# rrwick/Polypolish

Hardware: AMD Instinct MI355X
Metric: assembly Mbp polished/sec at 200x coverage; bit-identical FASTA vs reference (higher is better)
Workload: dtype u8/u32 counts + f64 depth

## Files before the change

polypolish_amd/__init__.py:

```python
from __future__ import annotations

import ctypes as C
import os

import numpy as np

HERE = os.path.dirname(os.path.abspath(__file__))
ROOT = os.path.dirname(HERE)
LIB_PATH = os.environ.get("PP_LIB_PATH") or os.path.join(HERE, "_build", "libpolypolish_hip.so")

OK, ERR_QUIT, ERR_HIP, ERR_ARG, ERR_LIMIT, ERR_PANIC = 0, 1, 3, 4, 5, 101
ERR_NOT_ASCII = 6
MEM_HOST, MEM_DEVICE, MEM_PEER = 0, 1, 2
STATUS = ("kept", "changed", "low_depth", "none", "multiple", "too_close")
OPS = "MIDNSHP=X"


class PolypolishError(RuntimeError):
    def __init__(self, code, msg):
        super().__init__(f"[{code}] {msg}")
        self.code, self.msg = code, msg


class Params(C.Structure):
# ... 1002 lines not shown
        run._keep = keep
        return run

    def result_size(self):
        n = C.c_uint64()
        self._chk(lib().pp_polish_result_size(self._h, C.byref(n)))
        return n.value

    def result_device_ptr(self):
        return lib().pp_polish_result_device(self._h)

    def result(self):
        n = self.result_size()
        out = np.zeros(max(n, 1), dtype=np.uint8)
        offs = np.zeros(self._n_contigs + 1, dtype=np.uint64)
        stats = (ContigStats * self._n_contigs)()
        self._chk(lib().pp_polish_result(self._h, out.ctypes.data, MEM_HOST, offs.ctypes.data, stats))
        st = [dict(polished_len=s.polished_len, changed=s.changed, zero_depth=s.zero_depth, depth_sum=s.depth_sum)
              for s in stats]
        return out[:n].tobytes(), offs, st

    def trust_mirrors(self, on=True):
        f = lib().pp_ctx_trust_mirrors_
        f.argtypes = [C.c_void_p, C.c_int]
        f.restype = C.c_int
        self._chk(f(self._h, int(bool(on))))

    def took_direct_path(self):
        return bool(lib().pp_polish_took_direct_path(self._h))

    def kernel_times(self):
        kt = KernelTimes()
        lib().pp_polish_kernel_times(self._h, C.byref(kt))
        return kt.as_dict()

    def first_kernel_ms(self):
        kt = getattr(self, "_kt", None)
        if kt is None:
            kt = self._kt = KernelTimes()
            self._kt_ref = C.byref(kt)
            self._kt_fn = lib().pp_polish_kernel_times
        self._kt_fn(self._h, self._kt_ref)
        return (kt.name[0], kt.ms[0]) if kt.n else None

    def positions(self):
        G = self._G
        arrs = {"depth": np.zeros(G, np.float64), "status": np.zeros(G, np.uint8)}
        for k in ("count_a", "count_c", "count_g", "count_t", "count_other", "valid_thr", "invalid_thr"):
            arrs[k] = np.zeros(G, np.uint32)
        po = PositionsOut(*[arrs[k].ctypes.data for k in ("depth", "count_a", "count_c", "count_g", "count_t",
                                                          "count_other", "valid_thr", "invalid_thr", "status")])
        self._chk(lib().pp_polish_positions(self._h, C.byref(po)))
        return arrs

    def debug_tsv(self, contig_names, lo=0, hi=None, chunk=64 << 20) -> bytes:
        names = [n.encode() if isinstance(n, str) else bytes(n) for n in contig_names]
        if len(names) != self._n_contigs:
            raise PolypolishError(ERR_ARG, "debug_tsv: one name per contig")
        arr = (C.c_char_p * max(len(names), 1))(*names)
        hi = self._G if hi is None else int(hi)
        buf = np.empty(max(int(chunk), 1), dtype=np.uint8)
        n, nxt = C.c_uint64(), C.c_uint64()
        parts, p = [], int(lo)
        while True:
            self._chk(lib().pp_polish_debug_tsv(self._h, C.cast(arr, C.c_void_p), p, hi, buf.ctypes.data, MEM_HOST, len(buf),
                                                C.byref(n), C.byref(nxt)))
            parts.append(buf[:n.value].tobytes())
# ... 130 lines not shown
```

polypolish_amd/csrc/pp_internal.h:

```cpp
#pragma once

#include <hip/hip_runtime.h>

#include <cstdarg>
#include <cstdint>
#include <cstdio>
#include <string>
#include <thread>
#include <vector>

#include "polypolish_hip.h"

#ifndef PP_MIRROR_REGISTRY_DECLARED
#define PP_MIRROR_REGISTRY_DECLARED
void pp_mirror_register_(const void *owner, const void *p, size_t bytes);
void pp_mirror_forget_(const void *owner);
bool pp_mirror_trusted_(const void *p, size_t bytes);
#endif

namespace pp {

constexpr int TILE = 2048;
constexpr int TILE_THREADS = 1024;
constexpr int COARSE_WINDOWS = 8;
// ... 28 lines not shown
    DE_LEN_MISMATCH = 2,
    DE_OUT_OF_BOUNDS = 3,
    DE_BAD_CONTIG = 4,
    DE_BAD_K = 5,
    DE_BAD_RUN = 6,
    DE_BAD_ENDS = 7,
    DE_NON_ASCII = 8,
    DE_INTERNAL = 9,
    DE_TOO_DEEP = 10,
    DE_OVERFLOW = 11,
    DE_CAPACITY = 12,
    DE_HALO = 14,
    DE_CAPACITY_LATE = 13,
    DE_BAD_MIRROR = 15,
    DE_MIRROR_ORDER = 16,
    DE_SEQ_RANGE = 18,
    DE_GW_HINT = 17,
};


enum MetaWord : uint32_t {
    MW_STATUS = 0,
    MW_COUNTERS = 1,
    MW_ITEMS = 3,
    MW_SCRATCH = 4,
    MW_OUT_BYTES = 5,
    MW_REPLAY_ITEMS = 6,
    MW_KEYS = 8,
    MW_MAXLEN = 9,
    MW_SCR_NEED = 10,
    MW_X_NEED = 12,
    MW_N_NEED = 13,
    MW_XMAT_ITEMS = 14,
    MW_CTG_OUT = 16,
};
enum MetaCounter : uint32_t {
    MC_LISTED = 0,
    MC_MULTI = 1,
    MC_FLAGGED = 2,
    MC_SLABS = 3,
};
constexpr size_t meta_stats_at(size_t nc) { return (size_t)MW_CTG_OUT + nc + 1; }
constexpr size_t meta_heavy_at(size_t nc) { return meta_stats_at(nc) + 3 * nc; }
constexpr size_t meta_words(size_t nc) { return meta_heavy_at(nc) + (HEAVY_WORDS + 1) / 2; }

struct MetaView {
    const uint64_t *w;
    uint64_t operator[](MetaWord i) const { return w[i]; }
    uint32_t counter(MetaCounter c) const { return (uint32_t)(w[MW_COUNTERS + c / 2] >> (32 * (c & 1))); }
    bool ok() const { return w[MW_STATUS] == ~0ull; }
};

struct DevBuf {
    void *p = nullptr;
    size_t cap = 0;
};

struct KernelTimer {
    const char *name;
    hipEvent_t start, stop;
};

struct ContigStatsDev {
    unsigned long long changed;
    unsigned long long zero_depth;
    unsigned long long depth_fx;
// ... 20 lines not shown
    uint32_t n_contigs = 0;
    std::vector<uint64_t> contig_off;
    uint64_t G = 0;
    pp_params params{};
    const uint8_t *d_bases = nullptr;
    pp_aln_batch dbatch{};
    bool have_batch = false;
    bool batch_borrowed = false;
    uint64_t acc_n = 0, acc_seq = 0, acc_cig = 0;
    uint64_t total_out = 0, n_multi = 0, n_keys = 0;
    uint64_t last_dev_error = ~0ull;
    std::vector<uint64_t> contig_out_off;
    std::vector<pp_contig_stats> stats;

    pp::DevBuf b_bases, b_contig_off, b_status;
    pp::DevBuf b_in[11];
    bool acc_wo = false;
    pp::DevBuf b_gstart, b_nkeep, b_aflag, b_hist, b_wincnt, b_winoff, b_entA, b_entB, b_ccnt, b_coff;
    pp::DevBuf b_code, b_winlen, b_winout, b_flag_pos, b_flag_cov, b_flag_scr, b_scratch;
    pp::DevBuf b_vote_tab;
    pp::DevBuf b_multi, b_meta, b_out, b_flag_bits, b_win_nflag, b_win_slab, b_slab_win, b_slabs, b_ents, b_keys, b_own;
    pp::DevBuf b_win_heavy, b_hslab;
    std::vector<uint64_t> wo_runs;
    pp::DevBuf b_runs, b_first, b_xcnt, b_xent, b_need_win, b_win_lo, b_win_hi;
    std::vector<uint32_t> runs_on_dev;
    size_t xcap = 0;
    bool no_direct = false;
    bool wo_untrusted = false;
    bool trust_all = false;
    bool no_wo = false;
    size_t xcap_limit = ~(size_t)0;
    uint32_t maxlen_hint = 0;
    bool last_direct = false;
    bool nothing_flagged_last = false;
    std::vector<uint32_t> emit;
    std::vector<uint32_t> run_full_of;
    uint32_t run_nc = 0;
    uint32_t last_multi = ~0u;
    uint32_t last_listed = ~0u;
    bool no_compact = false;
    uint64_t *h_meta = nullptr;
    pp::DevBuf b_wincoarse;
    pp::DevBuf b_emit_done;
    bool emit_done_clean = false;
    uint64_t *d_hmeta = nullptr;
    bool stream_may_be_busy = false;
    uint64_t emit_serial = 0;
    struct MetaReady {
        const void *meta; uint32_t words; const void *za, *zb, *zc; uint32_t nwin; const void *tab; double fv, fi; const void *ze;
        bool operator==(const MetaReady &o) const {
            return meta == o.meta && words == o.words && za == o.za && zb == o.zb && zc == o.zc && nwin == o.nwin && tab == o.tab && fv == o.fv && fi == o.fi && ze == o.ze;
        }
    };
    MetaReady meta_ready{};
    bool meta_ready_valid = false;
    size_t h_meta_words = 0;
    std::vector<uint8_t> own_blob;
    pp::DevBuf b_sub_bases;
    size_t cap_ent = 0, cap_scr = 0, cap_multi = 0, cap_out = 0, cap_flag = 0, cap_slabs = 0, cap_ents = 0, cap_keys = 0;
    pp::DevBuf b_dbg_depth, b_dbg_counts, b_dbg_status;
    bool job_debug = false;
    bool dfmt_ready = false;
    pp::DevBuf b_dfmt_idx, b_dfmt_rec;
    pp::DevBuf b_dfmt_names, b_dfmt_noff, b_dfmt_emit;
    pp::DevBuf b_dfmt_len, b_dfmt_bsum, b_dfmt_boff, b_dfmt_res, b_dfmt_stage;

// ... 45 lines not shown
```

polypolish_amd/csrc/pp_k_direct.h:

```cpp
#pragma once

#include "pp_wo_home.h"

namespace pp {

constexpr u32 NOHOME = 0xFFFFFFFFu;
__device__ __forceinline__ bool wo_bulk(bool contig_ok, u32 ref_start, u32 seq_len, u32 op0, u64 clen) {
    return contig_ok && op0 == ((seq_len << 4) | (u32)PP_OP_M) && seq_len > 0 && seq_len <= FAST_MAX_LEN && (u64)ref_start + seq_len <= clen;
}
__device__ __forceinline__ uint4 wo_item(u64 so, u32 len, u32 kc, u64 g, u32 w, u32 file_idx) {
    uint4 e;
    e.x = (u32)so;
    e.y = ((u32)(so >> 32) & 0xFFu) | (kc << 8) | (len << 24);
    e.z = (u32)(int)((long long)g - (long long)w * TILE) & 0x3FFFFFFFu;
    e.w = file_idx;
    return e;
}

constexpr u32 XLOCAL = 64, CTG_LDS = 1024;
struct CtgTab {
    const u64 *lds, *mem;
    bool in_lds;
    __device__ __forceinline__ u64 operator()(u32 i) const {
        u32 x, y;
        if (in_lds) {
            const u64 v = lds[i];
            x = (u32)v; y = (u32)(v >> 32);
            asm volatile("" : "+v"(x), "+v"(y));
        } else {
            const u64 v = mem[i];
            x = (u32)v; y = (u32)(v >> 32);
            asm volatile("" : "+v"(x), "+v"(y));
        }
        return (u64)x | ((u64)y << 32);
    }
    __device__ __forceinline__ void pair(u32 i, u64 &a, u64 &b) const {
        u32 x, y, z, w;
        if (in_lds) {
            const u64 v = lds[i], v1 = lds[i + 1u];
            x = (u32)v; y = (u32)(v >> 32); z = (u32)v1; w = (u32)(v1 >> 32);
            asm volatile("" : "+v"(x), "+v"(y), "+v"(z), "+v"(w));
        } else {
            const u64 v = mem[i], v1 = mem[i + 1u];
            x = (u32)v; y = (u32)(v >> 32); z = (u32)v1; w = (u32)(v1 >> 32);
            asm volatile("" : "+v"(x), "+v"(y), "+v"(z), "+v"(w));
        }
        a = (u64)x | ((u64)y << 32);
        b = (u64)z | ((u64)w << 32);
    }
};
struct XSink {
    uint4 *st_item;
    u32 *st_key;
    u32 *l_cnt, *l_base, *l_nb;
    u32 *n_st;
    u32 xstage, wbase, xcap;
    u32 *x_cnt, *x_nb;
    uint4 *xent;
    u64 *x_need, *status;
    __device__ __forceinline__ void put(u32 w, u32 slot, const uint4 &e) const {
        if (slot < xcap) xent[(u64)w * xcap + slot] = e;
        else {
            atomicMax(x_need, (u64)slot + 1ull);
            report(status, slot, DE_CAPACITY);
        }
    }
    __device__ __forceinline__ void emit(u32 w, const uint4 &e) const {
        const u32 wl = w - wbase;
        if (wl < XLOCAL) {
            const u32 pos = atomicAdd(n_st, 1u);
            if (pos < xstage) {
                st_key[pos] = (wl << 16) | atomicAdd(&l_cnt[wl], 1u);
                st_item[pos] = e;
                return;
            }
        }
        put(w, atomicAdd(&x_cnt[w], 1u), e);
    }
    __device__ __forceinline__ void not_bulk(u32 h) const {
        if (h - wbase < XLOCAL) atomicAdd(&l_nb[h - wbase], 1u); else atomicAdd(&x_nb[h], 1u);
    }
    __device__ __forceinline__ void clear() const {
        if (threadIdx.x < XLOCAL) { l_cnt[threadIdx.x] = 0; l_nb[threadIdx.x] = 0; }
        if (threadIdx.x == 0) *n_st = 0;
    }
    __device__ __forceinline__ void flush() const {
        __syncthreads();
        if (threadIdx.x < XLOCAL) {
            const u32 c = l_cnt[threadIdx.x], nb = l_nb[threadIdx.x];
            l_base[threadIdx.x] = c ? atomicAdd(&x_cnt[wbase + threadIdx.x], c) : 0u;
            if (nb) atomicAdd(&x_nb[wbase + threadIdx.x], nb);
        }
        __syncthreads();
        for (u32 i = threadIdx.x; i < min(*n_st, xstage); i += blockDim.x) {
            const u32 key = st_key[i], wl = key >> 16;
            put(wbase + wl, l_base[wl] + (key & 0xFFFFu), st_item[i]);
        }
    }
};

struct PrepdArgs {
    u64 n;
    const pp_wo_rec *wo;
    const u64 *cig_off;
    const u32 *n_cig, *cigar;
    const u8 *seq;
    const u64 *contig_off;
    u32 n_contigs, nwin;
    const u32 *run_end;
    u32 n_runs;
    u32 *first, *x_cnt, *x_nb;
    uint4 *xent;
    u32 xcap;
    u32 *maxlen;
    u64 *x_need;
    u64 unused_[3];
    u64 seq_bytes;
    u64 *status;
};

template <typename CTG>
__device__ __forceinline__ void general_record(const pp_wo_rec &r, const PrepdArgs &P, CTG ctg, const XSink &X) {
    u32 g_out = 0, nk_out = 0;
    u8 fl_out = 0;
    const u32 fi = r.file_idx;
    if (fi >= P.n) return;
    if (r.contig >= P.n_contigs) { report(P.status, fi, DE_BAD_CONTIG); return; }
    const u64 c_lo = ctg(r.contig), c_hi = ctg(r.contig + 1u);
    X.not_bulk(wo_home(c_lo, r.ref_start, P.nwin));
    {
        const bool multi = r.op0 == PP_WO_MULTI_RUN;
        const u32 sl = r.seq_len;
        const u8 *const sq = P.seq + r.seq_off;
        u64 tail8 = 0;
        if (sl >= 8u) __builtin_memcpy(&tail8, sq + (sl - 8u), 8);
        u32 nc = 1;
        u64 co = 0;
        if (multi) { nc = P.n_cig[fi]; co = P.cig_off[fi]; }
        if (nc == 0) report(P.status, fi, DE_BAD_RUN);
        else {
            const u32 *const cg = P.cigar + co;
            u32 r0 = r.op0, r1 = 0, r2 = 0, r3 = 0, r4 = 0, r5 = 0, r6 = 0, r7 = 0;
            if (multi) {
                r0 = cg[0];
                r1 = cg[min(1u, nc - 1u)]; r2 = cg[min(2u, nc - 1u)]; r3 = cg[min(3u, nc - 1u)]; r4 = cg[min(4u, nc - 1u)];
                r5 = cg[min(5u, nc - 1u)]; r6 = cg[min(6u, nc - 1u)]; r7 = cg[min(7u, nc - 1u)];
            }
            prep_general_t(fi, r.ref_start, sl, nc,
                           [&](u32 i) -> u32 {
// ... 1 lines not shown
                               const u32 a = (i & 1u) ? r1 : r0, b = (i & 1u) ? r3 : r2, c = (i & 1u) ? r5 : r4, d = (i & 1u) ? r7 : r6;
                               const u32 ab = (i & 2u) ? b : a, cd = (i & 2u) ? d : c;
                               return (i & 4u) ? cd : ab;
                           },
                           [&](u32 i) -> u8 { return sl >= 8u && i + 8u >= sl ? (u8)(tail8 >> (8u * (i + 8u - sl))) : sq[i]; },
                           c_lo, c_hi - c_lo, &g_out, &nk_out, &fl_out, P.status);
        }
    }
    const u32 word = nk_out | ((u32)fl_out << 30);
    if (!word) return;
    const u32 kc = kclass_of(r.k);
    const u32 cls = word >> 30, ia = (word >> 9) & 0xFFu, idel = (word >> 17) & 1u;
    for_each_piece(g_out, word, [&](u32 piece, u32 g, u32 sp) {
        if (!sp) return;
        const u32 wa = g / (u32)TILE, wb = min((g + sp - 1u) / (u32)TILE, P.nwin - 1u);
        u64 pso = r.seq_off;
        u32 len = sp, fl = 0, zf = 0;
        if (cls == NKW_INDEL1) {
            if (piece == 0u) zf = 1u;
            else if (piece == 1u) { zf = 2u; pso += ia - 1u + idel; len = idel ? 0u : 2u; }
            else pso += idel ? ia : ia + 1u;
        } else fl = cls;
        for (u32 w = wa; w <= wb && w >= wa; w++) {
            uint4 e;
            e.x = fl ? sp : (u32)pso;
            e.y = (fl ? 0u : (((u32)(pso >> 32) & 0xFFu) | (len << 24))) | (kc << 8) | (fl << 16);
            e.z = ((u32)(int)((long long)g - (long long)w * TILE) & 0x3FFFFFFFu) | (zf << 30);
            e.w = fi;
            X.emit(w, e);
        }
    });
}

template <int THREADS>
__global__ __launch_bounds__(THREADS, PP_PREP_WAVES) void k_prepd(u64 chunk, PrepdArgs P) {
    constexpr u32 LATER_MAX = THREADS >= 1024 ? 768 : 320, XSTAGE = 2 * THREADS;
    __shared__ uint4 later[2 * LATER_MAX];
    __shared__ u32 n_later, s_unit;
    __shared__ uint4 st_item[XSTAGE];
    __shared__ u32 st_key[XSTAGE], l_cnt[XLOCAL], l_base[XLOCAL], l_nb[XLOCAL], n_st, s_wbase;
    __shared__ u64 s_ctg[CTG_LDS + 1];
    PP_STAMP(0, 0);
    const u64 n = P.n;
    const pp_wo_rec *const wo = P.wo;
    const u32 n_contigs = P.n_contigs, nwin = P.nwin, n_runs = P.n_runs;
    __shared__ u32 s_run_end[PP_WO_MAX_RUNS];
    if (threadIdx.x < P.n_runs) s_run_end[threadIdx.x] = P.run_end[threadIdx.x];
    const u32 *const run_end = s_run_end;
    u64 *const status = P.status;
    const u64 lo = (u64)blockIdx.x * chunk, hi = min(n, lo + chunk);
    const bool ctg_lds = n_contigs <= CTG_LDS;
    if (ctg_lds)
        for (u32 i = threadIdx.x; i <= n_contigs; i += blockDim.x) s_ctg[i] = P.contig_off[i];
    if (threadIdx.x == 0) {
        n_later = 0;
        s_unit = blockDim.x >> 6;
        u32 wb = 0;
        if (lo < hi) {
            const pp_wo_rec r0 = wo[lo];
            if (r0.contig < n_contigs) wb = wo_home(P.contig_off[r0.contig], r0.ref_start, nwin);
        }
        s_wbase = wb;
    }
    XSink X{st_item, st_key, l_cnt, l_base, l_nb, &n_st, XSTAGE, 0u, P.xcap, P.x_cnt, P.x_nb, P.xent, P.x_need, status};
    X.clear();
    __syncthreads();
    PP_STAMP(0, 1);
    X.wbase = s_wbase;
    const CtgTab ctg{s_ctg, P.contig_off, ctg_lds};
    const u32 lane = threadIdx.x & 63u;
    const u32 stride = nwin + 1u;
    u32 *const first = P.first;
    auto fill = [&](bool want, u32 run, u32 from, u32 to, u32 val) {
        if (want && to - from < 4u) {
            for (u32 w = from; w <= to; w++) first[(u64)run * stride + w] = val;
            want = false;
        }
        u64 m = __ballot(want);
        while (m) {
            const int lead = __ffsll((long long)m) - 1;
            m &= m - 1;
            const u32 rr = (u32)__builtin_amdgcn_readlane((int)run, lead), ff = (u32)__builtin_amdgcn_readlane((int)from, lead),
                      tt = (u32)__builtin_amdgcn_readlane((int)to, lead), vv = (u32)__builtin_amdgcn_readlane((int)val, lead);
            for (u64 w = (u64)ff + lane; w <= tt; w += 64) first[(u64)rr * stride + w] = vv;
        }
    };
    u32 runw = 0, runw_lo = 0;
    u32 fast_len = 0;
    constexpr int WU = PP_WO_UNROLL;
    const uint4 *wq = (const uint4 *)wo;
    const u64 trip = (u64)WU * blockDim.x;
    const u64 span = (hi - lo + trip - 1) / trip * trip;
#ifndef PP_PREPD_DYN
#define PP_PREPD_DYN 1
#endif
    const u32 ustride = PP_PREPD_DYN ? 64u : blockDim.x;
    uint4 qa[WU], qb[WU];
    u32 pc[WU], pr[WU];
    auto ask = [&](int u, u64 a0, bool real) __attribute__((always_inline)) {
        const u64 a = real ? min(a0 + (u64)u * ustride, n - 1) : lo;
        qa[u] = wq[2 * a];
        qb[u] = wq[2 * a + 1];
        const u64 wf = a0 - lane + (u64)u * ustride;
        const u64 pf = real ? min(wf ? wf - 1 : 0, n - 1) : lo;
        pc[u] = wo[pf].contig;
        pr[u] = wo[pf].ref_start;
    };
#ifndef PP_PREPD_ROLL
#define PP_PREPD_ROLL 1
#endif
    const u32 n_units = (u32)(span / (64u * WU));
    auto unit_a0 = [&](u32 j) -> u64 { return lo + (u64)j * (64u * WU) + lane; };
    u32 unit = (u32)__builtin_amdgcn_readfirstlane((int)(threadIdx.x >> 6));
    if (PP_PREPD_ROLL) {
#pragma unroll
        for (int u = 0; u < WU; u++) ask(u, PP_PREPD_DYN ? unit_a0(unit) : lo + threadIdx.x, true);
    }
    for (u64 a0 = lo + threadIdx.x; PP_PREPD_DYN ? unit < n_units : a0 < lo + span; a0 += trip) {
        u32 unit_next = 0;
        if (PP_PREPD_DYN) {
            a0 = unit_a0(unit);
            u32 t = 0;
            if (lane == 0) t = atomicAdd(&s_unit, 1u);
            unit_next = (u32)__builtin_amdgcn_readfirstlane((int)t);
        }
        if (!PP_PREPD_ROLL) {
#pragma unroll
            for (int u = 0; u < WU; u++) ask(u, a0, true);
// ... 22 lines not shown
                while (run + 1u < n_runs && (u32)a >= run_end[run]) { run_lo = run_end[run]; run++; run_hi = run_end[run]; }
            const bool valid = h != NOHOME, starts = (u32)a == run_lo;
            const bool begins = valid && (starts || (hp != NOHOME && h > hp));
            const bool descent = valid && !starts && hp != NOHOME && h < hp;
            const bool ends = valid && (u32)a + 1u == run_hi;
            const bool bad = in && (file_idx >= n || k == 0 || seq_off + seq_len > (1ull << 40) || seq_off + seq_len > P.seq_bytes);
            if (__ballot(begins || descent || ends || bad)) {
                if (bad) {
                    if (file_idx >= n) report(status, a, DE_BAD_MIRROR);
                    else if (k == 0) report(status, file_idx, DE_BAD_K);
                    else if (seq_off + seq_len > (1ull << 40)) report(status, file_idx, DE_OVERFLOW);
                    else report(status, file_idx, DE_SEQ_RANGE);
                }
                if (descent) report(status, (1ull << 40) - 1ull, DE_MIRROR_ORDER);
                fill(begins, run, starts ? 0u : hp + 1u, h, (u32)a);
                fill(ends, run, h + 1u, nwin, (u32)a + 1u);
            }
            const u32 w1 = bulk ? (u32)((g + seq_len - 1u) / (u64)TILE) : 0u;
            if (bulk && w1 > h) X.emit(w1, wo_item(seq_off, seq_len, kclass_of(k), g, w1, file_idx));
            if (bulk) fast_len = max(fast_len, seq_len);
            else if (in) {
                const u32 slot = atomicAdd(&n_later, 1u);
                if (slot < LATER_MAX) { later[2u * slot] = qa[u]; later[2u * slot + 1u] = qb[u]; }
            }
            if (PP_PREPD_ROLL) ask(u, a0_next, more);
        }
        unit = unit_next;
    }
    PP_STAMP(0, 2);
    __syncthreads();
    PP_STAMP(0, 3);
    const u32 n_noted = n_later;
    const bool listed = n_noted <= LATER_MAX;
    if (listed) {
        for (u32 i = threadIdx.x; i < n_noted; i += blockDim.x) {
            const uint4 qa = later[2u * i], qb = later[2u * i + 1u];
            pp_wo_rec r;
            r.contig = qa.x; r.ref_start = qa.y; r.k = qa.z; r.seq_len = qa.w;
            r.seq_off = (u64)qb.x | ((u64)qb.y << 32); r.op0 = qb.z; r.file_idx = qb.w;
            general_record(r, P, ctg, X);
        }
    }
    if (!listed && n_noted) {
        for (u64 a = lo + threadIdx.x; a < hi; a += blockDim.x) {
            const pp_wo_rec r = wo[a];
            const u32 cc = min(r.contig, n_contigs - 1u);
            if (!wo_bulk(r.contig < n_contigs, r.ref_start, r.seq_len, r.op0, ctg(cc + 1u) - ctg(cc))) general_record(r, P, ctg, X);
        }
    }
    PP_STAMP(0, 4);
    X.flush();
    PP_STAMP(0, 5);
    if (__ballot(fast_len > PLAIN_NARROW_MAX)) {
        for (int o = 32; o > 0; o >>= 1) fast_len = max(fast_len, (u32)__shfl_xor((int)fast_len, o, 64));
        if (lane == 0 && fast_len > __hip_atomic_load(P.maxlen, __ATOMIC_RELAXED, __HIP_MEMORY_SCOPE_AGENT)) atomicMax(P.maxlen, fast_len);
    }
    PP_STAMP(0, 6);
}

__global__ __launch_bounds__(256) void k_winplan(u32 nwin, u32 n_runs, const u32 *__restrict__ first, const u32 *__restrict__ x_cnt,
                                                 const u32 *__restrict__ x_nb, u32 xcap, u32 heavy_min, u32 *__restrict__ heavy, u8 *__restrict__ win_heavy,
                                                 u64 *__restrict__ n_items, u64 *status) {
    const u32 w = blockIdx.x * blockDim.x + threadIdx.x;
    const bool live = w < nwin && *status == ~0ull;
    u32 cnt = 0;
    bool bad = false;
    if (live) {
        cnt = min(x_cnt[w], xcap);
        for (u32 r = 0; r < n_runs; r++) {
            const u32 a = first[(u64)r * (nwin + 1u) + w], b = first[(u64)r * (nwin + 1u) + w + 1u];
            if (b < a) bad = true; else cnt += b - a;
        }
        if (!bad) cnt -= min(cnt, x_nb[w]);
        if (bad) report(status, (1ull << 40) - 1ull, DE_MIRROR_ORDER);
        else {
            if (cnt >= MAX_BUCKET) report(status, w, DE_TOO_DEEP);
            note_heavy(w, cnt, heavy_min, heavy, win_heavy);
        }
    } else if (w < nwin) win_heavy[w] = 0;
    const u32 tot = wave_sum(bad ? 0u : cnt);
    if ((threadIdx.x & 63u) == 0 && tot) atomicAdd(n_items, (u64)tot);
}

__global__ __launch_bounds__(1024) void k_xmat(const u32 *__restrict__ need_win, const u64 *__restrict__ n_need, u32 nwin,
// ... 52 lines not shown
```

polypolish_amd/csrc/pp_kernels.hip:

```cpp
#include "pp_internal.h"

#include <algorithm>
#include <cstring>

#include "pp_k_common.h"
#include "pp_k_prep.h"
#include "pp_k_bucket.h"
#include "pp_k_direct.h"
#include "pp_k_tile.h"
#include "pp_k_exact.h"
#include "pp_k_emit.h"
#include "pp_k_debug.h"
#include <hip/hip_ext.h>

using namespace pp;

static bool env_is0(const char *name) { const char *v = getenv(name); return v && atoi(v) == 0; }
static bool env_on(const char *name) { const char *v = getenv(name); return v && atoi(v) != 0; }
static long env_num(const char *name, long dflt) { const char *v = getenv(name); return v ? atol(v) : dflt; }
struct Knobs {
    bool timer_record = env_on("PP_TIMER_RECORD");
    bool no_seq4 = env_is0("PP_SEQ4");
    bool no_wo = env_is0("PP_WO");
    bool no_direct = env_is0("PP_DIRECT");
    uint64_t xent_budget = getenv("PP_XENT_BUDGET") ? strtoull(getenv("PP_XENT_BUDGET"), nullptr, 10) : (8ull << 30);
    int bucket_levels = (int)env_num("PP_BUCKET_LEVELS", 0);
    long fill_range = env_num("PP_FILL_RANGE", 0);
    bool no_init_ahead = env_is0("PP_INIT_AHEAD");
    long heavy_min = env_num("PP_HEAVY_MIN", 0);
    bool check_wo = env_on("PP_CHECK_WO");
    long prepd_blocks = env_num("PP_PREPD_BLOCKS", 0);
    long prepd_threads = env_num("PP_PREPD_THREADS", 1024);
    bool debug_replay2 = env_on("PP_DEBUG_REPLAY2");
    bool no_speculate = env_is0("PP_SPECULATE");
    bool result_copy = env_on("PP_RESULT_COPY");
    bool sync_wait = getenv("PP_SYNC") && strcmp(getenv("PP_SYNC"), "poll") != 0;
    bool sync_query = getenv("PP_SYNC") && !strcmp(getenv("PP_SYNC"), "query");
    bool no_emit_fuse = env_is0("PP_EMIT_FUSE");
    bool trace_flagged = getenv("PP_TRACE_FLAGGED") != nullptr;
    bool timing = getenv("PP_TIMING") != nullptr;
    const char *prep_stamps_file = getenv("PP_PREP_STAMPS_FILE"), *tile_stamps_file = getenv("PP_TILE_STAMPS_FILE");
};
static const Knobs &knobs() {
    static const Knobs k;
    return k;
}

namespace pp {

int dev_ensure(pp_ctx *ctx, DevBuf &b, size_t bytes) {
    if (bytes == 0) bytes = 16;
    if (b.cap >= bytes) return PP_OK;
    if (b.p) {
        PP_HIPCHK(ctx, hipStreamSynchronize(ctx->stream));
        PP_HIPCHK(ctx, hipFree(b.p));
        b.p = nullptr;
        b.cap = 0;
    }
    size_t want = bytes + bytes / 8 + 256;
    PP_HIPCHK(ctx, hipMalloc(&b.p, want));
    b.cap = want;
    return PP_OK;
}

void dev_free(DevBuf &b) {
// ... 607 lines not shown
static int check_mirror(pp_ctx *ctx, const RunPlan &P, const RunDev &D) {
    const pp_aln_batch &B = ctx->dbatch;
    const uint64_t n = P.n;
    const bool check_wo = knobs().check_wo || (ctx->wo_untrusted && !ctx->trust_all);
    if (!(check_wo && B.wo && !knobs().no_wo && !ctx->no_wo && n)) return PP_OK;
    if (int rc = dev_ensure(ctx, ctx->b_aflag, (size_t)((n + 31) / 32) * 4)) return rc;
    PP_HIPCHK(ctx, hipMemsetAsync(ctx->b_aflag.p, 0, (size_t)((n + 31) / 32) * 4, ctx->stream));
    hipLaunchKernelGGL(k_check_wo, dim3((unsigned)((n + 255) / 256)), dim3(256), 0, ctx->stream, (u64)n, B.wo, B.contig, B.ref_start, B.k,
                       (const u64 *)B.seq_off, B.seq_len, (const u64 *)B.cig_off, B.n_cig, B.cigar, (u32 *)ctx->b_aflag.p, D.status());
    return PP_OK;
}

#ifdef PP_PREP_STAMPS
static DevBuf b_pstamps;
constexpr size_t pstamp_bytes = (size_t)2 * 16384 * 64;
static int prep_stamps_begin(pp_ctx *ctx) {
    if (int rc = dev_ensure(ctx, b_pstamps, pstamp_bytes)) return rc;
    PP_HIPCHK(ctx, hipMemsetAsync(b_pstamps.p, 0, pstamp_bytes, ctx->stream));
    u64 *sp = (u64 *)b_pstamps.p;
    PP_HIPCHK(ctx, hipMemcpyToSymbolAsync(HIP_SYMBOL(pp::g_prep_stamps), &sp, sizeof sp, 0, hipMemcpyHostToDevice, ctx->stream));
    return PP_OK;
}
static int prep_stamps_dump(pp_ctx *ctx) {
    const char *path = knobs().prep_stamps_file;
    if (!path) return PP_OK;
    std::vector<uint64_t> hs(pstamp_bytes / 8);
    PP_HIPCHK(ctx, hipMemcpyAsync(hs.data(), b_pstamps.p, pstamp_bytes, hipMemcpyDeviceToHost, ctx->stream));
    PP_HIPCHK(ctx, hipStreamSynchronize(ctx->stream));
    if (FILE *f = fopen(path, "wb")) { fwrite(hs.data(), 1, pstamp_bytes, f); fclose(f); }
    return PP_OK;
}
#endif

static void prep_direct(pp_ctx *ctx, const RunPlan &P, const RunDev &D) {
    const Knobs &K = knobs();
    const pp_aln_batch &B = ctx->dbatch;
    const uint64_t n = P.n;
    const u32 nwin = P.nwin;
    hipStream_t st = ctx->stream;
    const uint64_t noted_est = B.n_cig_total > n ? (B.n_cig_total - n) / 2 : 0;
    const uint64_t nbd_default = std::max<uint64_t>(std::max<uint64_t>(768, n / 8700), noted_est / 400);
    const uint32_t NBD = (uint32_t)std::max<uint64_t>(1, std::min<uint64_t>(K.prepd_blocks > 0 ? (uint64_t)K.prepd_blocks : nbd_default, (n + 2047) / 2048));
    const uint64_t chunk_d = (n + NBD - 1) / NBD;
    timer_begin(ctx, "prep");
    PrepdArgs PA{};
    PA.n = n; PA.wo = D.wo; PA.cig_off = (const u64 *)B.cig_off; PA.n_cig = B.n_cig; PA.cigar = B.cigar; PA.seq = B.seq;
    PA.contig_off = (const u64 *)ctx->b_contig_off.p; PA.n_contigs = P.nc_full; PA.nwin = nwin;
    PA.run_end = (const u32 *)ctx->b_runs.p; PA.n_runs = P.n_runs; PA.first = (u32 *)ctx->b_first.p;
    PA.x_cnt = (u32 *)ctx->b_xcnt.p; PA.x_nb = (u32 *)ctx->b_xcnt.p + nwin; PA.xent = (uint4 *)ctx->b_xent.p; PA.xcap = (u32)ctx->xcap;
    PA.maxlen = (u32 *)(D.meta + MW_MAXLEN); PA.x_need = D.meta + MW_X_NEED;
    PA.seq_bytes = B.seq_bytes;
    PA.status = D.status();
    if (K.prepd_threads == 1024) hipLaunchKernelGGL(k_prepd<1024>, dim3(NBD), dim3(1024), 0, st, (u64)chunk_d, PA);
    else hipLaunchKernelGGL(k_prepd<512>, dim3(NBD), dim3(512), 0, st, (u64)chunk_d, PA);
    timer_end(ctx);
    timer_begin(ctx, "bucket");
    hipLaunchKernelGGL(k_winplan, dim3((nwin + 255) / 256), dim3(256), 0, st, nwin, P.n_runs, (const u32 *)ctx->b_first.p,
                       (const u32 *)ctx->b_xcnt.p, (const u32 *)ctx->b_xcnt.p + nwin, (u32)ctx->xcap, P.heavy_min, D.heavy, (u8 *)ctx->b_win_heavy.p,
                       D.meta + MW_ITEMS, D.status());
    timer_end(ctx);
}

static void prep_bucketing(pp_ctx *ctx, const RunPlan &P, const RunDev &D) {
    const pp_aln_batch &B = ctx->dbatch;
    const uint64_t n = P.n, chunk = P.chunk;
    const u32 nwin = P.nwin, NB = P.NB, nranges = P.nranges, cw = P.cw, ncoarse = P.ncoarse, ncranges = P.ncranges, frange = P.frange, heavy_min = P.heavy_min;
    hipStream_t st = ctx->stream;
    const pp_wo_rec *const d_wo = D.wo;
    u64 *const d_status = D.status();
    u32 *const d_heavy = D.heavy;
    u8 *const d_win_heavy = (u8 *)ctx->b_win_heavy.p;
    u32 *d_gstart = (u32 *)ctx->b_gstart.p, *d_nkeep = (u32 *)ctx->b_nkeep.p;
    u32 *d_hist = (u32 *)ctx->b_hist.p, *d_wincnt = (u32 *)ctx->b_wincnt.p, *d_winoff = (u32 *)ctx->b_winoff.p;
    uint4 *d_entA = (uint4 *)ctx->b_entA.p, *d_entB = (uint4 *)ctx->b_entB.p;
    u32 *d_ccnt = (u32 *)ctx->b_ccnt.p, *d_coff = (u32 *)ctx->b_coff.p;
    timer_begin(ctx, "prep");
#define PP_PREP_ARGS dim3(NB), dim3(1024), 0, st, (u64)n, (u64)chunk, d_wo, B.contig, B.ref_start, (const u64 *)B.seq_off, B.seq_len, \
                     (const u64 *)B.cig_off, B.n_cig, B.cigar, B.seq, (const u64 *)ctx->b_contig_off.p, P.nc_full, D.gbase, D.slice, D.own_full, \
                     d_gstart, d_nkeep, (u32 *)(D.meta + MW_MAXLEN), nwin, cw, ncoarse
    if (!P.fused_count) {
        if (d_wo) hipLaunchKernelGGL((k_prep<false, true>), PP_PREP_ARGS, (u32 *)nullptr, d_status);
        else hipLaunchKernelGGL((k_prep<false, false>), PP_PREP_ARGS, (u32 *)nullptr, d_status);
    } else {
        if (d_wo) hipLaunchKernelGGL((k_prep<true, true>), PP_PREP_ARGS, d_hist, d_status);
        else hipLaunchKernelGGL((k_prep<true, false>), PP_PREP_ARGS, d_hist, d_status);
    }
#undef PP_PREP_ARGS
// ... 400 lines not shown
            if (need <= cap) return;
            if (trace) fprintf(stderr, "[timing] pass %d: %s %zu -> need %llu\n", attempt + 1, what, cap, (unsigned long long)need);
            cap = (size_t)(need + need / 8 + 1024);
            grew = true;
        };
        const uint64_t x_need = M[MW_X_NEED];
        grow(ctx->cap_ent, ctx->last_direct ? M[MW_XMAT_ITEMS] : M[MW_ITEMS], "work items");
        if (ctx->last_direct && x_need > ctx->xcap) {
            if (x_need + x_need / 8 + 1024 > ctx->xcap_limit) {
                if (trace) fprintf(stderr, "[timing] pass %d: a window needs %llu extras (room for %zu at most) -> bucketing path\n", attempt + 1,
                                   (unsigned long long)x_need, ctx->xcap_limit);
                ctx->no_direct = true;
                grew = true;
            } else grow(ctx->xcap, x_need, "extras per window");
        }
        const bool list_full = M.counter(MC_LISTED) > ctx->cap_flag;
        grow(ctx->cap_flag, std::min<uint64_t>(M.counter(MC_LISTED), G), "listed positions");
        grow(ctx->cap_scr, M[MW_SCR_NEED], "replay scratch");
        grow(ctx->cap_multi, M.counter(MC_MULTI) + (list_full ? std::min<uint64_t>(M.counter(MC_LISTED), G) : 0), "multi-byte winners");
        grow(ctx->cap_slabs, M.counter(MC_SLABS), "tally slabs");
        grow(ctx->cap_ents, M[MW_REPLAY_ITEMS], "ordered replay items");
        if (ctx->debug) grow(ctx->cap_keys, M[MW_KEYS], "key records");
        grow(ctx->cap_out, M[MW_OUT_BYTES], "polished bytes");
        if (!grew) return ctx->fail(PP_ERR_HIP, "device reported a capacity overflow that the host cannot locate");
    }
    const MetaView M{meta.data()};
    ctx->total_out = M[MW_OUT_BYTES];
    ctx->last_listed = M.counter(MC_LISTED);
    ctx->nothing_flagged_last = M.counter(MC_LISTED) == 0 && M.counter(MC_FLAGGED) == 0;
    ctx->maxlen_hint = (uint32_t)M[MW_MAXLEN];
    ctx->n_multi = M.counter(MC_MULTI);
    ctx->last_multi = M.counter(MC_MULTI);
    ctx->n_keys = M[MW_KEYS];
    const uint32_t rnc = ctx->run_nc;
    const uint64_t *r_out = M.w + MW_CTG_OUT;
    const ContigStatsDev *hs = (const ContigStatsDev *)(M.w + meta_stats_at(rnc));
    ctx->contig_out_off.assign((size_t)nc + 1, 0);
    ctx->stats.assign(nc, pp_contig_stats{0, 0, 0, 0.0});
    uint32_t j = 0;
    for (uint32_t c = 0; c < nc; c++) {
        ctx->contig_out_off[c] = r_out[j];
        const bool mine = ctx->run_full_of.empty() || (j < rnc && ctx->run_full_of[j] == c);
        if (!mine) continue;
        ctx->stats[c].polished_len = r_out[j + 1] - r_out[j];
        ctx->stats[c].changed = hs[j].changed;
        ctx->stats[c].zero_depth = hs[j].zero_depth;
        ctx->stats[c].depth_sum = (double)hs[j].depth_fx / (double)(1u << DEPTH_FX_BITS);
        j++;
    }
    ctx->contig_out_off[nc] = r_out[rnc];
    if (ctx->profiling) {
        timers_collect(ctx, &ctx->last_times);
        ctx->last_times.n_entries = n_entries;
        ctx->last_times.n_flagged = M.counter(MC_FLAGGED);
        ctx->last_times.n_passes = (uint64_t)attempt + 1;
    }
    ctx->job_done = true;
    ctx->job_debug = ctx->debug;
    ctx->job_open = false;
    return PP_OK;
}

extern "C" int pp_polish_result_size(pp_ctx *ctx, uint64_t *total_bytes) {
    if (!ctx || !total_bytes) return PP_ERR_ARG;
    if (!ctx->job_done) return ctx->fail(PP_ERR_ARG, "no finished polish job");
    *total_bytes = ctx->total_out;
// ... 195 lines not shown
            }
            return ctx->fail(PP_ERR_LIMIT, "a --debug line longer than %llu bytes", (unsigned long long)DFMT_STAGE);
        }
        if (host && bytes) {
            PP_HIPCHK(ctx, hipMemcpyAsync(out + written, ctx->b_dfmt_stage.p, bytes, hipMemcpyDeviceToHost, st));
            PP_HIPCHK(ctx, hipStreamSynchronize(st));
        }
        written += bytes;
        p += n_fit;
        if (n_fit < N && room == caller_room) break;
    }
    *len = written;
    *pos_next = p;
    return PP_OK;
}

extern "C" void *pp_host_pinned_alloc_(pp_ctx *ctx, uint64_t bytes) {
    void *p = nullptr;
    if (!ctx || pp_ctx_wait(ctx) != PP_OK || hipSetDevice(ctx->device) != hipSuccess) return nullptr;
    return hipHostMalloc(&p, bytes, hipHostMallocDefault) == hipSuccess ? p : nullptr;
}
extern "C" void pp_host_pinned_free_(void *p) {
    if (p) (void)hipHostFree(p);
}

extern "C" int pp_ctx_set_profiling(pp_ctx *ctx, int enable) {
    if (!ctx) return PP_ERR_ARG;
    if (int rdy = pp_ctx_wait(ctx)) return rdy;
    ctx->profiling = enable == 2 ? 2 : (enable != 0);
    return PP_OK;
}

extern "C" int pp_polish_took_direct_path(const pp_ctx *ctx) { return ctx && ctx->last_direct ? 1 : 0; }

extern "C" int pp_polish_kernel_times(pp_ctx *ctx, pp_kernel_times *out) {
    if (!ctx || !out) return PP_ERR_ARG;
    *out = ctx->last_times;
    return PP_OK;
}

extern "C" void pp_tokenize_warm_(hipStream_t st);
extern "C" void pp_filter_warm_(hipStream_t st);
__global__ void k_warm(uint32_t *p) {
    if (p) p[threadIdx.x] = 0;
}

static int device_init(pp_ctx *ctx) {
    int n = 0;
    if (hipGetDeviceCount(&n) != hipSuccess || n <= 0) return PP_ERR_HIP;
    if (ctx->device < 0 || ctx->device >= n) return PP_ERR_ARG;
    if (hipSetDevice(ctx->device) != hipSuccess) return PP_ERR_HIP;
    if (hipStreamCreateWithFlags(&ctx->stream, hipStreamNonBlocking) != hipSuccess) return PP_ERR_HIP;
    return PP_OK;
}

extern "C" int pp_device_count(void) {
    int n = 0;
    return hipGetDeviceCount(&n) == hipSuccess && n > 0 ? n : 0;
}

extern "C" int pp_ctx_create(int device, pp_ctx **out) {
    if (!out) return PP_ERR_ARG;
    *out = nullptr;
    pp_ctx *ctx = new pp_ctx();
    ctx->device = device;
    const int rc = device_init(ctx);
// ... 116 lines not shown
```

Baseline: 18190.

## Retune k_prepd to smaller blocks, u32 contig table, and round-based replay of noted records

The k_prepd kernel moves from a 1024/512-thread template to a fixed 512-thread build with a smaller LDS stage, and stores the contig offset table in LDS as 32-bit values to cut shared memory. Noted records are replayed in rounds of 192 threads, with a flush after each round so the stage never overflows. Block count and chunk size are re-derived so more, smaller workgroups are launched. Overflow counters are added to the meta words and exposed for diagnostics. The u32 contig table assumes genome offsets fit in 32 bits, and the per-round syncs add overhead.

```diff
diff --git a/polypolish_amd/__init__.py b/polypolish_amd/__init__.py
--- a/polypolish_amd/__init__.py
+++ b/polypolish_amd/__init__.py
@@ -1058,7 +1058,13 @@
     def kernel_times(self):
         kt = KernelTimes()
         lib().pp_polish_kernel_times(self._h, C.byref(kt))
-        return kt.as_dict()
+        out = kt.as_dict()
+        f = getattr(lib(), "pp_polish_prepd_overflows_", None)
+        if f is not None:
+            lists, stage = C.c_uint32(0), C.c_uint32(0)
+            f(self._h, C.byref(lists), C.byref(stage))
+            out["prepd_list_overflows"], out["prepd_stage_misses"] = lists.value, stage.value
+        return out
 
     def first_kernel_ms(self):
         kt = getattr(self, "_kt", None)
diff --git a/polypolish_amd/csrc/pp_internal.h b/polypolish_amd/csrc/pp_internal.h
--- a/polypolish_amd/csrc/pp_internal.h
+++ b/polypolish_amd/csrc/pp_internal.h
@@ -84,6 +84,7 @@
     MW_X_NEED = 12,
     MW_N_NEED = 13,
     MW_XMAT_ITEMS = 14,
+    MW_PREPD_OVF = 15,
     MW_CTG_OUT = 16,
 };
 enum MetaCounter : uint32_t {
@@ -170,6 +171,7 @@
     size_t xcap_limit = ~(size_t)0;
     uint32_t maxlen_hint = 0;
     bool last_direct = false;
+    uint32_t prepd_list_ovf = 0, prepd_stage_miss = 0;
     bool nothing_flagged_last = false;
     std::vector<uint32_t> emit;
     std::vector<uint32_t> run_full_of;
diff --git a/polypolish_amd/csrc/pp_k_direct.h b/polypolish_amd/csrc/pp_k_direct.h
--- a/polypolish_amd/csrc/pp_k_direct.h
+++ b/polypolish_amd/csrc/pp_k_direct.h
@@ -19,14 +19,14 @@
 
 constexpr u32 XLOCAL = 64, CTG_LDS = 1024;
 struct CtgTab {
-    const u64 *lds, *mem;
+    const u32 *lds;
+    const u64 *mem;
     bool in_lds;
     __device__ __forceinline__ u64 operator()(u32 i) const {
         u32 x, y;
         if (in_lds) {
-            const u64 v = lds[i];
-            x = (u32)v; y = (u32)(v >> 32);
-            asm volatile("" : "+v"(x), "+v"(y));
+            x = lds[i]; y = 0;
+            asm volatile("" : "+v"(x));
         } else {
             const u64 v = mem[i];
             x = (u32)v; y = (u32)(v >> 32);
@@ -37,9 +37,8 @@
     __device__ __forceinline__ void pair(u32 i, u64 &a, u64 &b) const {
         u32 x, y, z, w;
         if (in_lds) {
-            const u64 v = lds[i], v1 = lds[i + 1u];
-            x = (u32)v; y = (u32)(v >> 32); z = (u32)v1; w = (u32)(v1 >> 32);
-            asm volatile("" : "+v"(x), "+v"(y), "+v"(z), "+v"(w));
+            x = lds[i]; z = lds[i + 1u]; y = 0; w = 0;
+            asm volatile("" : "+v"(x), "+v"(z));
         } else {
             const u64 v = mem[i], v1 = mem[i + 1u];
             x = (u32)v; y = (u32)(v >> 32); z = (u32)v1; w = (u32)(v1 >> 32);
@@ -58,6 +57,7 @@
     u32 *x_cnt, *x_nb;
     uint4 *xent;
     u64 *x_need, *status;
+    u32 *ovf;
     __device__ __forceinline__ void put(u32 w, u32 slot, const uint4 &e) const {
         if (slot < xcap) xent[(u64)w * xcap + slot] = e;
         else {
@@ -74,6 +74,7 @@
                 st_item[pos] = e;
                 return;
             }
+            atomicAdd(&ovf[1], 1u);
         }
         put(w, atomicAdd(&x_cnt[w], 1u), e);
     }
@@ -88,8 +89,10 @@
         __syncthreads();
         if (threadIdx.x < XLOCAL) {
             const u32 c = l_cnt[threadIdx.x], nb = l_nb[threadIdx.x];
-            l_base[threadIdx.x] = c ? atomicAdd(&x_cnt[wbase + threadIdx.x], c) : 0u;
-            if (nb) atomicAdd(&x_nb[wbase + threadIdx.x], nb);
+            u32 w = wbase + threadIdx.x;
+            asm volatile("" : "+v"(w));
+            l_base[threadIdx.x] = c ? atomicAdd(&x_cnt[w], c) : 0u;
+            if (nb) atomicAdd(&x_nb[w], nb);
         }
         __syncthreads();
         for (u32 i = threadIdx.x; i < min(*n_st, xstage); i += blockDim.x) {
@@ -114,7 +117,8 @@
     u32 xcap;
     u32 *maxlen;
     u64 *x_need;
-    u64 unused_[3];
+    u32 *ovf;
+    u64 unused_[2];
     u64 seq_bytes;
     u64 *status;
 };
@@ -182,14 +186,18 @@
     });
 }
 
-template <int THREADS>
-__global__ __launch_bounds__(THREADS, PP_PREP_WAVES) void k_prepd(u64 chunk, PrepdArgs P) {
-    constexpr u32 LATER_MAX = THREADS >= 1024 ? 768 : 320, XSTAGE = 2 * THREADS;
+#ifndef PP_PREPD_T
+#define PP_PREPD_T 512
+#endif
+constexpr u32 PREPD_THREADS = PP_PREPD_T, PREPD_LATER_MAX = 640, PREPD_XSTAGE = 768, PREPD_ROUND = 192;
+static_assert(PREPD_ROUND <= PREPD_THREADS && PREPD_ROUND % 64 == 0 && 4 * PREPD_ROUND <= PREPD_XSTAGE, "a round's pieces fit the stage");
+__global__ __launch_bounds__(PREPD_THREADS, PP_PREP_WAVES) void k_prepd(u64 chunk, PrepdArgs P) {
+    constexpr u32 LATER_MAX = PREPD_LATER_MAX, XSTAGE = PREPD_XSTAGE, ROUND = PREPD_ROUND;
     __shared__ uint4 later[2 * LATER_MAX];
     __shared__ u32 n_later, s_unit;
     __shared__ uint4 st_item[XSTAGE];
     __shared__ u32 st_key[XSTAGE], l_cnt[XLOCAL], l_base[XLOCAL], l_nb[XLOCAL], n_st, s_wbase;
-    __shared__ u64 s_ctg[CTG_LDS + 1];
+    __shared__ u32 s_ctg[CTG_LDS + 1];
     PP_STAMP(0, 0);
     const u64 n = P.n;
     const pp_wo_rec *const wo = P.wo;
@@ -201,7 +209,7 @@
     const u64 lo = (u64)blockIdx.x * chunk, hi = min(n, lo + chunk);
     const bool ctg_lds = n_contigs <= CTG_LDS;
     if (ctg_lds)
-        for (u32 i = threadIdx.x; i <= n_contigs; i += blockDim.x) s_ctg[i] = P.contig_off[i];
+        for (u32 i = threadIdx.x; i <= n_contigs; i += blockDim.x) s_ctg[i] = (u32)P.contig_off[i];
     if (threadIdx.x == 0) {
         n_later = 0;
         s_unit = blockDim.x >> 6;
@@ -212,7 +220,7 @@
         }
         s_wbase = wb;
     }
-    XSink X{st_item, st_key, l_cnt, l_base, l_nb, &n_st, XSTAGE, 0u, P.xcap, P.x_cnt, P.x_nb, P.xent, P.x_need, status};
+    XSink X{st_item, st_key, l_cnt, l_base, l_nb, &n_st, XSTAGE, 0u, P.xcap, P.x_cnt, P.x_nb, P.xent, P.x_need, status, P.ovf};
     X.clear();
     __syncthreads();
     PP_STAMP(0, 1);
@@ -237,13 +245,14 @@
     };
     u32 runw = 0, runw_lo = 0;
     u32 fast_len = 0;
+#ifndef PP_PREPD_DYN
+#define PP_PREPD_DYN 1
+#endif
     constexpr int WU = PP_WO_UNROLL;
     const uint4 *wq = (const uint4 *)wo;
     const u64 trip = (u64)WU * blockDim.x;
-    const u64 span = (hi - lo + trip - 1) / trip * trip;
-#ifndef PP_PREPD_DYN
-#define PP_PREPD_DYN 1
-#endif
+    const u64 grain = PP_PREPD_DYN ? (u64)WU * 64u : trip;
+    const u64 span = (hi - lo + grain - 1) / grain * grain;
     const u32 ustride = PP_PREPD_DYN ? 64u : blockDim.x;
     uint4 qa[WU], qb[WU];
     u32 pc[WU], pr[WU];
@@ -332,24 +341,35 @@
     PP_STAMP(0, 3);
     const u32 n_noted = n_later;
     const bool listed = n_noted <= LATER_MAX;
-    if (listed) {
-        for (u32 i = threadIdx.x; i < n_noted; i += blockDim.x) {
-            const uint4 qa = later[2u * i], qb = later[2u * i + 1u];
-            pp_wo_rec r;
-            r.contig = qa.x; r.ref_start = qa.y; r.k = qa.z; r.seq_len = qa.w;
-            r.seq_off = (u64)qb.x | ((u64)qb.y << 32); r.op0 = qb.z; r.file_idx = qb.w;
-            general_record(r, P, ctg, X);
-        }
-    }
-    if (!listed && n_noted) {
-        for (u64 a = lo + threadIdx.x; a < hi; a += blockDim.x) {
-            const pp_wo_rec r = wo[a];
-            const u32 cc = min(r.contig, n_contigs - 1u);
-            if (!wo_bulk(r.contig < n_contigs, r.ref_start, r.seq_len, r.op0, ctg(cc + 1u) - ctg(cc))) general_record(r, P, ctg, X);
-        }
-    }
-    PP_STAMP(0, 4);
-    X.flush();
+    if (!listed && threadIdx.x == 0) atomicAdd(&P.ovf[0], 1u);
+    const u32 rounds = listed ? (n_noted + ROUND - 1u) / ROUND : 1u;
+    for (u32 rd = 0;; rd++) {
+        if (rd == rounds) PP_STAMP(0, 4);
+        X.flush();
+        if (rd == rounds) break;
+        __syncthreads();
+        X.clear();
+        __syncthreads();
+        if (listed) {
+            const u32 i = rd * ROUND + threadIdx.x;
+            if (threadIdx.x < ROUND && i < n_noted) {
+                const uint4 qa = later[2u * i], qb = later[2u * i + 1u];
+                pp_wo_rec r;
+                r.contig = qa.x; r.ref_start = qa.y; r.k = qa.z; r.seq_len = qa.w;
+                r.seq_off = (u64)qb.x | ((u64)qb.y << 32); r.op0 = qb.z; r.file_idx = qb.w;
+                general_record(r, P, ctg, X);
+            }
+        } else {
+            u32 blk = blockIdx.x;
+            asm volatile("" : "+s"(blk));
+            const u64 lo2 = (u64)blk * chunk, hi2 = min(P.n, lo2 + chunk);
+            for (u64 a = lo2 + threadIdx.x; a < hi2; a += blockDim.x) {
+                const pp_wo_rec r = P.wo[a];
+                const u32 cc = min(r.contig, n_contigs - 1u);
+                if (!wo_bulk(r.contig < n_contigs, r.ref_start, r.seq_len, r.op0, ctg(cc + 1u) - ctg(cc))) general_record(r, P, ctg, X);
+            }
+        }
+    }
     PP_STAMP(0, 5);
     if (__ballot(fast_len > PLAIN_NARROW_MAX)) {
         for (int o = 32; o > 0; o >>= 1) fast_len = max(fast_len, (u32)__shfl_xor((int)fast_len, o, 64));
diff --git a/polypolish_amd/csrc/pp_kernels.hip b/polypolish_amd/csrc/pp_kernels.hip
--- a/polypolish_amd/csrc/pp_kernels.hip
+++ b/polypolish_amd/csrc/pp_kernels.hip
@@ -30,7 +30,6 @@
     long heavy_min = env_num("PP_HEAVY_MIN", 0);
     bool check_wo = env_on("PP_CHECK_WO");
     long prepd_blocks = env_num("PP_PREPD_BLOCKS", 0);
-    long prepd_threads = env_num("PP_PREPD_THREADS", 1024);
     bool debug_replay2 = env_on("PP_DEBUG_REPLAY2");
     bool no_speculate = env_is0("PP_SPECULATE");
     bool result_copy = env_on("PP_RESULT_COPY");
@@ -704,6 +703,10 @@
 }
 #endif
 
+#ifndef PP_PREPD_CHUNK
+#define PP_PREPD_CHUNK 4340
+#endif
+constexpr uint64_t PREPD_MIN_BLOCKS = 1536, PREPD_CHUNK = PP_PREPD_CHUNK;
 static void prep_direct(pp_ctx *ctx, const RunPlan &P, const RunDev &D) {
     const Knobs &K = knobs();
     const pp_aln_batch &B = ctx->dbatch;
@@ -711,9 +714,10 @@
     const u32 nwin = P.nwin;
     hipStream_t st = ctx->stream;
     const uint64_t noted_est = B.n_cig_total > n ? (B.n_cig_total - n) / 2 : 0;
-    const uint64_t nbd_default = std::max<uint64_t>(std::max<uint64_t>(768, n / 8700), noted_est / 400);
-    const uint32_t NBD = (uint32_t)std::max<uint64_t>(1, std::min<uint64_t>(K.prepd_blocks > 0 ? (uint64_t)K.prepd_blocks : nbd_default, (n + 2047) / 2048));
-    const uint64_t chunk_d = (n + NBD - 1) / NBD;
+    const uint64_t nbd_default = std::max<uint64_t>(std::max<uint64_t>(PREPD_MIN_BLOCKS, n / PREPD_CHUNK), noted_est / (PREPD_LATER_MAX / 2));
+    const uint64_t nbd_want = std::max<uint64_t>(1, std::min<uint64_t>(K.prepd_blocks > 0 ? (uint64_t)K.prepd_blocks : nbd_default, (n + 2047) / 2048));
+    const uint64_t chunk_d = (n + nbd_want - 1) / nbd_want;
+    const uint32_t NBD = (uint32_t)((n + chunk_d - 1) / chunk_d);
     timer_begin(ctx, "prep");
     PrepdArgs PA{};
     PA.n = n; PA.wo = D.wo; PA.cig_off = (const u64 *)B.cig_off; PA.n_cig = B.n_cig; PA.cigar = B.cigar; PA.seq = B.seq;
@@ -721,10 +725,10 @@
     PA.run_end = (const u32 *)ctx->b_runs.p; PA.n_runs = P.n_runs; PA.first = (u32 *)ctx->b_first.p;
     PA.x_cnt = (u32 *)ctx->b_xcnt.p; PA.x_nb = (u32 *)ctx->b_xcnt.p + nwin; PA.xent = (uint4 *)ctx->b_xent.p; PA.xcap = (u32)ctx->xcap;
     PA.maxlen = (u32 *)(D.meta + MW_MAXLEN); PA.x_need = D.meta + MW_X_NEED;
+    PA.ovf = (u32 *)(D.meta + MW_PREPD_OVF);
     PA.seq_bytes = B.seq_bytes;
     PA.status = D.status();
-    if (K.prepd_threads == 1024) hipLaunchKernelGGL(k_prepd<1024>, dim3(NBD), dim3(1024), 0, st, (u64)chunk_d, PA);
-    else hipLaunchKernelGGL(k_prepd<512>, dim3(NBD), dim3(512), 0, st, (u64)chunk_d, PA);
+    hipLaunchKernelGGL(k_prepd, dim3(NBD), dim3(PREPD_THREADS), 0, st, (u64)chunk_d, PA);
     timer_end(ctx);
     timer_begin(ctx, "bucket");
     hipLaunchKernelGGL(k_winplan, dim3((nwin + 255) / 256), dim3(256), 0, st, nwin, P.n_runs, (const u32 *)ctx->b_first.p,
@@ -1191,6 +1195,11 @@
     ctx->n_multi = M.counter(MC_MULTI);
     ctx->last_multi = M.counter(MC_MULTI);
     ctx->n_keys = M[MW_KEYS];
+    ctx->prepd_list_ovf = (uint32_t)M[MW_PREPD_OVF];
+    ctx->prepd_stage_miss = (uint32_t)(M[MW_PREPD_OVF] >> 32);
+    if (trace && ctx->last_direct)
+        fprintf(stderr, "[timing] %u work items; k_prepd: %u workgroups walked their entries twice (list of noted records full), %u extras found the LDS stage full\n",
+                n_entries, ctx->prepd_list_ovf, ctx->prepd_stage_miss);
     const uint32_t rnc = ctx->run_nc;
     const uint64_t *r_out = M.w + MW_CTG_OUT;
     const ContigStatsDev *hs = (const ContigStatsDev *)(M.w + meta_stats_at(rnc));
@@ -1452,6 +1461,12 @@
 }
 
 extern "C" int pp_polish_took_direct_path(const pp_ctx *ctx) { return ctx && ctx->last_direct ? 1 : 0; }
+extern "C" int pp_polish_prepd_overflows_(const pp_ctx *ctx, uint32_t *lists, uint32_t *stage) {
+    if (!ctx || !lists || !stage) return PP_ERR_ARG;
+    *lists = ctx->prepd_list_ovf;
+    *stage = ctx->prepd_stage_miss;
+    return PP_OK;
+}
 
 extern "C" int pp_polish_kernel_times(pp_ctx *ctx, pp_kernel_times *out) {
     if (!ctx || !out) return PP_ERR_ARG;
```

After: 18330, median of 5. Within noise of the previous version (+0.8%).
